# prestodb/presto

Measured on AMD Instinct MI355X. Metric: tpch_lineitem_rows_per_sec, higher is better.
Workload: dtype f64; 1 GPU; TPC-H SF100 Q1 & Q3 on 1xMI355X - one step = one Q1 pass + one Q3 pass, columns resident in HBM; query=q1+q3, rows_per_gpu=1200075804, mode=f64

## Files before the change

### include/presto_gpu.h

```cpp
#ifndef PRESTO_GPU_H
#define PRESTO_GPU_H
#include <stdint.h>

#ifdef __cplusplus
extern "C" {
#endif

#define PG_ABI_VERSION 1

typedef int32_t pg_status;
#define PG_OK 0
#define PG_ERR (-1)
const char* pg_last_error(void);

pg_status pg_device_count(int32_t* out);
pg_status pg_device_sync(void);
pg_status pg_device_malloc(int64_t bytes, void** out);
pg_status pg_device_free(void* p);
pg_status pg_memcpy_h2d(void* dst, const void* src, int64_t bytes);
pg_status pg_memcpy_d2h(void* dst, const void* src, int64_t bytes);
pg_status pg_memcpy_d2d(void* dst, const void* src, int64_t bytes);
double pg_last_hot_kernel_ms(void);
double pg_hot_max_ms(void);
void pg_hot_reset(void);
int64_t pg_q1_fast_launches(void);
int64_t pg_build_staged_launches(void);

typedef enum {
    PG_T_U8 = 0,
    PG_T_I32 = 1,
    PG_T_I64 = 2,
    PG_T_F64 = 3,
    PG_T_I128 = 5,
    PG_T_VARBIN = 4,
} pg_type;

typedef struct {
    int32_t tag;
    int32_t on_device;
    void* data;
    const uint8_t* null_mask;
    const int32_t* offsets;
    const int32_t* dict_ids;
    int32_t dict_n;
} pg_col;

typedef struct {
    int64_t n_rows;
    int32_t n_cols;
    pg_col cols[32];
} pg_page;


typedef enum { PG_CMP_LT = 0, PG_CMP_LE, PG_CMP_GT, PG_CMP_GE, PG_CMP_EQ,
               PG_CMP_NE,
               PG_CMP_CONTAINS, PG_CMP_PREFIX,
               PG_CMP_CONTAINS2, PG_CMP_NOT_CONTAINS2,
               PG_CMP_IS_NULL, PG_CMP_IS_NOT_NULL } pg_cmp;

// ... 230 lines not shown
```

### presto_amd/csrc/kernels.hip

```cpp
#include <hip/hip_runtime.h>
#include <stdio.h>
#include <stdlib.h>
#include <string.h>
#include <map>
#include <vector>
#include <algorithm>
#include <type_traits>
#include <stdexcept>
#include <string>

#include "../../include/presto_gpu.h"
#include "fixed128.h"
#include "sortkey.h"

static __thread char g_err[512];
extern "C" const char* pg_last_error(void) { return g_err; }
static pg_status seterr(const char* msg)
{
    snprintf(g_err, sizeof(g_err), "%s", msg);
    return PG_ERR;
}
#define CHK(x)                                                          \
    do {                                                                \
        hipError_t e_ = (x);                                            \
// ... 87 lines not shown
static hipEvent_t g_ev0, g_ev1;
static bool g_ev_init = false;
static void hot_begin()
{
    hipError_t e;
    if (!g_ev_init) {
        e = hipEventCreate(&g_ev0);
        e = hipEventCreate(&g_ev1);
        g_ev_init = true;
    }
    e = hipEventRecord(g_ev0, g_stream);
    (void)e;
}
static void hot_end()
{
    hipError_t e;
    e = hipEventRecord(g_ev1, g_stream);
    e = hipEventSynchronize(g_ev1);
    float ms = 0;
    e = hipEventElapsedTime(&ms, g_ev0, g_ev1);
    (void)e;
    g_last_hot_ms = ms;
    if (ms > g_hot_max_ms) g_hot_max_ms = ms;
}
extern "C" double pg_last_hot_kernel_ms(void) { return g_last_hot_ms; }
extern "C" double pg_hot_max_ms(void) { return g_hot_max_ms; }
extern "C" void pg_hot_reset(void) { g_hot_max_ms = 0.0; }
static int64_t g_q1_fast_launches = 0;
extern "C" int64_t pg_q1_fast_launches(void) { return g_q1_fast_launches; }
static int64_t g_build_staged_launches = 0;
extern "C" int64_t pg_build_staged_launches(void)
{
    return g_build_staged_launches;
}

#define WAVE 64
#define FT_NBLOCKS 4096
#define FT_NTHREADS 256
#define FT_VL ((int64_t)FT_NBLOCKS * FT_NTHREADS)
static const int64_t TBL_EMPTY = INT64_MIN;

__device__ __host__ inline uint8_t d_tbl_tag(uint64_t h)
{
    return (uint8_t)((h >> 56) | 1);
}

__device__ inline double d_load_f64(const pg_col& c, int64_t i)
{
    switch (c.tag) {
        case PG_T_F64: return ((const double*)c.data)[i];
        case PG_T_I64: return (double)((const int64_t*)c.data)[i];
        case PG_T_I32: return (double)((const int32_t*)c.data)[i];
        default: return (double)((const uint8_t*)c.data)[i];
    }
}
__device__ inline int64_t d_load_i64(const pg_col& c, int64_t i)
{
    switch (c.tag) {
        case PG_T_I64: return ((const int64_t*)c.data)[i];
        case PG_T_I32: return (int64_t)((const int32_t*)c.data)[i];
        case PG_T_U8: return (int64_t)((const uint8_t*)c.data)[i];
        default: return (int64_t)((const double*)c.data)[i];
    }
}

__device__ inline int32_t d_find(const uint8_t* d, int32_t n,
// ... 1592 lines not shown
__device__ inline int64_t d_tbl_find_tagged(const int64_t* keys,
                                            const uint8_t* tags,
                                            int64_t mask, int64_t lmask,
                                            int32_t pbits, int64_t key)
{
    if (!tags) return d_tbl_find(keys, mask, lmask, pbits, key);
    uint64_t h = pg_murmur3_finalize(pg_bigint_hash(key));
    int64_t s = (int64_t)(h & (uint64_t)mask);
    uint8_t tag = d_tbl_tag(h);
    for (;;) {
        uint8_t t = tags[s];
        if (t == 0) return -1;
        if (t == tag && (keys[s] >> pbits) == key) return s;
        s = d_probe_next(s, lmask);
    }
}

struct slot_acc {
    unsigned long long dec;
    unsigned long long flo;
    unsigned long long fhi;
    unsigned long long cnt;
};

__device__ inline void d_atomic_add_dec_ck(unsigned long long* slot,
                                           int64_t ticks,
                                           unsigned long long* ovf)
{
    long long old = (long long)atomicAdd(slot, (unsigned long long)ticks);
    long long nv = old + ticks;
    if (((old ^ nv) & (ticks ^ nv)) < 0 && ovf) atomicAdd(ovf, 1ull);
}

__global__ __launch_bounds__(256) void k_probe_agg(
    pg_page pg, pg_plan_lookup_join plan, const int64_t* keys,
    const uint8_t* tags, int64_t mask, int64_t lmask, int32_t pbits,
    const unsigned long long* kbits, int64_t bmax,
    unsigned long long* acc, int32_t aw,
    unsigned long long* ovf )
{
    const int C = 4;
    int64_t base =
        ((int64_t)blockIdx.x * blockDim.x + threadIdx.x) * C;
    const int64_t stride = (int64_t)gridDim.x * blockDim.x * C;
    for (; base < pg.n_rows; base += stride) {
        const int64_t lim = base + C < pg.n_rows ? base + C : pg.n_rows;
        int64_t cur_key = 0, cur_slot = -2;
        int64_t run_dec = 0;
        long long run_min = INT64_MAX;
        uint64_t run_flo = 0, run_fhi = 0;
        int run_cnt = 0;
        auto flush = [&]() {
            if (cur_slot < 0 || run_cnt == 0) return;
            unsigned long long* s = acc + (size_t)cur_slot * aw;
            if (plan.dec_min) {
                atomicMin((long long*)&s[0], run_min);
            } else if (run_dec) {
                d_atomic_add_dec_ck(&s[0], run_dec, ovf);
            }
            if (!plan.dec_only && !plan.dec_min && (run_flo | run_fhi)) {
                unsigned long long old = atomicAdd(&s[1], run_flo);
                atomicAdd(&s[2],
                          run_fhi + (old > ~run_flo ? 1ull : 0ull));
            }
            atomicAdd(&s[aw - 1], (unsigned long long)run_cnt);
        };
        for (int64_t i = base; i < lim; i++) {
            if (!d_eval_preds(pg, plan.preds, plan.n_preds, i)) continue;
            int64_t key = d_load_i64(pg.cols[plan.key_col], i);
            if (cur_slot == -2 || key != cur_key) {
                flush();
                cur_key = key;
                if (!keys)
                    cur_slot = (uint64_t)(key - 1) <= (uint64_t)mask
                                   ? key - 1
                                   : -1;
                else
                    cur_slot = kbits && !d_kbit_test(kbits, bmax, key)
                                   ? -1
                                   : d_tbl_find_tagged(keys, tags, mask,
                                                       lmask, pbits, key);
                run_dec = 0;
                run_flo = run_fhi = 0;
                run_cnt = 0;
                run_min = INT64_MAX;
            }
            if (cur_slot < 0) continue;
            pg_agg ag;
            ag.proj = plan.proj;
            ag.dec_scale = plan.dec_scale;
            int64_t ticks = d_eval_proj_dec(pg, ag, i);
            if (plan.dec_min) {
                run_min = ticks < run_min ? ticks : run_min;
            } else if (__builtin_add_overflow(run_dec, ticks, &run_dec)) {
                if (ovf) atomicAdd(ovf, 1ull);
            }
            if (!plan.dec_only && !plan.dec_min) {
                double p = d_eval_proj_f64(pg, plan.proj, i);
                uint64_t phi, plo;
                d_fx128_from_f64_ck(p, &phi, &plo, ovf + 1);
                uint64_t nlo = run_flo + plo;
                run_fhi += phi + (nlo < plo ? 1u : 0u);
                run_flo = nlo;
            }
            run_cnt++;
        }
        flush();
    }
}

__global__ __launch_bounds__(256) void k_probe_agg_q3(
    const int32_t* sd , int32_t pred_op,
    int32_t pred_val, const int64_t* okey, const double* ep,
    const double* dc, int64_t n, const int64_t* keys, const uint8_t* tags,
    int64_t mask, int64_t lmask, int32_t pbits,
    const unsigned long long* kbits, int64_t bmax, int32_t dec_only,
    unsigned long long* acc, int32_t aw, unsigned long long* ovf)
{
    typedef int vi2 __attribute__((ext_vector_type(2)));
    typedef long vl2 __attribute__((ext_vector_type(2)));
    const int Q = 2;
    int64_t base0 = Q * ((int64_t)blockIdx.x * blockDim.x + threadIdx.x);
    int64_t stride = Q * (int64_t)gridDim.x * blockDim.x;
    for (int64_t base = base0; base < n; base += stride) {
        int64_t k[Q];
        int32_t s[Q];
        bool sel[Q];
        if (base + Q <= n) {
            vl2 ka = __builtin_nontemporal_load((const vl2*)(okey + base));
            k[0] = ka[0]; k[1] = ka[1];
            if (sd) {
                vi2 ss = __builtin_nontemporal_load((const vi2*)(sd + base));
                s[0] = ss[0]; s[1] = ss[1];
            }
#pragma unroll
            for (int j = 0; j < Q; j++) sel[j] = true;
        } else {
#pragma unroll
            for (int j = 0; j < Q; j++) {
                sel[j] = base + j < n;
                k[j] = sel[j] ? okey[base + j] : 0;
                s[j] = sel[j] && sd ? sd[base + j] : 0;
            }
        }
        if (sd) {
#pragma unroll
            for (int j = 0; j < Q; j++)
                sel[j] = sel[j] && (pred_op == PG_CMP_GT ? s[j] > pred_val
                                                         : s[j] < pred_val);
        }
        int64_t slot[Q];
#pragma unroll
        for (int j = 0; j < Q; j++) {
            slot[j] = -1;
            if (!sel[j]) continue;
            if (kbits && !d_kbit_test(kbits, bmax, k[j])) continue;
            uint64_t h = pg_murmur3_finalize(pg_bigint_hash(k[j]));
            int64_t p = (int64_t)(h & (uint64_t)mask);
            uint8_t tg = tags ? d_tbl_tag(h) : 0;
            for (;;) {
                if (tags) {
                    uint8_t t = tags[p];
                    if (t == 0) break;
                    if (t == tg && (keys[p] >> pbits) == k[j]) {
                        slot[j] = p;
                        break;
                    }
                } else {
                    int64_t kw = keys[p];
                    if (kw == TBL_EMPTY) break;
                    if ((kw >> pbits) == k[j]) { slot[j] = p; break; }
                }
                p = d_probe_next(p, lmask);
            }
        }
#pragma unroll
        for (int j = 0; j < Q; j++) {
            int64_t sl = slot[j];
            if (sl < 0) continue;
            double e = ep[base + j], d = dc[base + j];
            int64_t cents = d_round_ticks(e * 100.0);
            int64_t di = d_round_ticks(d * 100.0);
            int64_t ticks = cents * (100 - di);
            unsigned long long* s = acc + (size_t)sl * aw;
            atomicAdd(&s[0], (unsigned long long)ticks);
            if (!dec_only) {
                double pr = e * (1.0 - d);
                uint64_t phi, plo;
                d_fx128_from_f64_ck(pr, &phi, &plo, ovf + 1);
                unsigned long long old = atomicAdd(&s[1], plo);
                atomicAdd(&s[2], phi + (old > ~plo ? 1ull : 0ull));
            }
            atomicAdd(&s[aw - 1], 1ull);
        }
    }
}

__global__ __launch_bounds__(256) void k_probe_agg_pay(
    pg_page pg, pg_plan_lookup_join plan, const int64_t* keys1,
    const uint8_t* tags1, const int32_t* head1, int64_t mask1,
    int64_t lmask1, const unsigned long long* kbits1, int64_t bmax1,
    const int64_t* pay1, const int64_t* keys2,
    const uint8_t* tags2, int64_t mask2, int64_t lmask2,
    unsigned long long* acc2, int32_t aw, unsigned long long* ovf)
{
    int64_t i = (int64_t)blockIdx.x * blockDim.x + threadIdx.x;
    int64_t stride = (int64_t)gridDim.x * blockDim.x;
    for (; i < pg.n_rows; i += stride) {
        if (!d_eval_preds(pg, plan.preds, plan.n_preds, i)) continue;
        int64_t key = d_load_i64(pg.cols[plan.key_col], i);
        if (kbits1 && !d_kbit_test(kbits1, bmax1, key)) continue;
        int64_t s1 = d_tbl_find_tagged(keys1, tags1, mask1, lmask1, 0,
                                       key);
        if (s1 < 0) continue;
        int64_t r = head1 ? (int64_t)head1[s1] : s1;
        if (r < 0) continue;
        int64_t g = pay1[r];
        int64_t s2 =
            keys2 ? d_tbl_find_tagged(keys2, tags2, mask2, lmask2, 0, g)
                  : ((uint64_t)(g - 1) <= (uint64_t)mask2 ? g - 1 : -1);
        if (s2 < 0) continue;
        pg_agg ag;
        ag.proj = plan.proj;
        ag.dec_scale = plan.dec_scale;
        int64_t ticks = d_eval_proj_dec(pg, ag, i);
        unsigned long long* s = acc2 + (size_t)s2 * aw;
        d_atomic_add_dec_ck(&s[0], ticks, ovf);
        if (!plan.dec_only) {
// ... 823 lines not shown
                (int64_t)s[acc_words - 1];
        }
        __syncthreads();
        if (threadIdx.x == 0)
            running += wcnt[0] + wcnt[1] + wcnt[2] + wcnt[3];
        __syncthreads();
    }
}

__global__ __launch_bounds__(256) void k_groups_count(
    const unsigned long long* acc, int64_t stride_w, int64_t cnt_off,
    int32_t cnt_shift, unsigned long long cnt_mask,
    int64_t cap, int64_t chunk, int64_t* block_counts)
{
    const int64_t lo = (int64_t)blockIdx.x * chunk;
    const int64_t hi = min(lo + chunk, cap);
    const int lane = threadIdx.x & 63, wid = threadIdx.x >> 6;
    int64_t cnt = 0;
    for (int64_t base = lo + 64 * wid; base < hi; base += 256) {
        int64_t i = base + lane;
        bool sel = i < hi &&
                   ((acc[i * stride_w + cnt_off] >> cnt_shift) &
                    cnt_mask) > 0;
        uint64_t m = d_ballot(sel);
        if (lane == 0) cnt += __popcll(m);
    }
    __shared__ int64_t lds[4];
    if (lane == 0) lds[wid] = cnt;
    __syncthreads();
    if (threadIdx.x == 0)
        block_counts[blockIdx.x] = lds[0] + lds[1] + lds[2] + lds[3];
}

__global__ __launch_bounds__(256) void k_groups_emit(
    const int64_t* keys, const int32_t* head,
    const unsigned long long* acc, int32_t aw, build_payloads bp,
    int64_t cap, int64_t chunk, unsigned long long* cursor,
    int64_t* out_key, emit_outs payload_outs, int64_t* out_dec,
    double* out_f64, int64_t* out_cnt)
{
    const int64_t lo = (int64_t)blockIdx.x * chunk;
    const int64_t hi = min(lo + chunk, cap);
    const int lane = threadIdx.x & 63, wid = threadIdx.x >> 6;
    __shared__ int64_t wcnt[4];
    __shared__ int64_t running;
    {
        int64_t mycnt = 0;
        for (int64_t i = lo + threadIdx.x; i < hi; i += 256)
            mycnt += acc[i * aw + aw - 1] > 0;
        mycnt = d_bfly_i64(mycnt);
        if (lane == 0) wcnt[wid] = mycnt;
        __syncthreads();
        if (threadIdx.x == 0)
            running = wcnt[0] + wcnt[1] + wcnt[2] + wcnt[3]
                          ? (int64_t)atomicAdd(
                                cursor, (unsigned long long)(wcnt[0] +
                                                             wcnt[1] +
                                                             wcnt[2] +
                                                             wcnt[3]))
                          : 0;
    }
    __syncthreads();
    for (int64_t base = lo; base < hi; base += 256) {
        int64_t i = base + 64 * wid + lane;
        bool sel = i < hi && acc[i * aw + aw - 1] > 0;
        uint64_t m = d_ballot(sel);
        int wsum = __popcll(m);
        if (lane == 0) wcnt[wid] = wsum;
        __syncthreads();
        int64_t woff = running;
        for (int w = 0; w < wid; w++) woff += wcnt[w];
        if (sel) {
            int64_t pos = woff + __popcll(m & ((1ull << lane) - 1));
            int64_t kw = keys ? keys[i] : i + 1;
            out_key[pos] = bp.pack_bits ? (kw >> bp.pack_bits) : kw;
            int64_t r = bp.by_slot ? i : (int64_t)head[i];
            for (int o = 0; o < bp.n; o++) {
                int64_t pv = bp.pack_bits && o == 0
                                 ? (kw & ((1ll << bp.pack_bits) - 1))
                                 : 0;
                switch (bp.tag[o]) {
                    case PG_T_U8:
                        ((uint8_t*)payload_outs.ptr[o])[pos] =
                            bp.pack_bits && o == 0
                                ? (uint8_t)pv
                                : ((const uint8_t*)bp.ptr[o])[r];
                        break;
                    case PG_T_I32:
                        ((int32_t*)payload_outs.ptr[o])[pos] =
                            bp.pack_bits && o == 0
                                ? (int32_t)pv
                                : ((const int32_t*)bp.ptr[o])[r];
                        break;
                    case PG_T_I64:
                        ((int64_t*)payload_outs.ptr[o])[pos] =
                            bp.pack_bits && o == 0
                                ? pv
                                : ((const int64_t*)bp.ptr[o])[r];
                        break;
                    default:
                        ((double*)payload_outs.ptr[o])[pos] =
                            ((const double*)bp.ptr[o])[r];
                }
            }
            const unsigned long long* s = acc + (size_t)i * aw;
            out_dec[pos] = (int64_t)s[0];
            out_f64[pos] = aw == 4 ? fx128_to_f64(s[2], s[1]) : 0.0;
            out_cnt[pos] = (int64_t)s[aw - 1];
        }
        __syncthreads();
        if (threadIdx.x == 0)
            running += wcnt[0] + wcnt[1] + wcnt[2] + wcnt[3];
        __syncthreads();
    }
}

#define TOPN_NB 256
#define TOPN_MAXL 16

struct topn_cand {
    int64_t val_bits;
    int64_t key;
    int32_t date;
    int32_t valid;
};

__device__ inline bool d_topn_less(bool is_f64, int64_t av, int32_t ad,
                                   int64_t ak, int64_t bv, int32_t bd,
                                   int64_t bk)
{
    if (av != bv) {
        if (is_f64) {
            double x = __longlong_as_double(av), y = __longlong_as_double(bv);
            return x < y;
        }
        return av < bv;
    }
    if (ad != bd) return ad > bd;
    return ak > bk;
}

__global__ __launch_bounds__(256) void k_topn(const void* vals, int is_f64,
                                              const int32_t* dates,
                                              const int64_t* keys, int64_t n,
                                              int32_t L, topn_cand* block_out)
{
    int64_t lv[TOPN_MAXL];
// ... 984 lines not shown
                bufs.emplace_back();
                bufs.back().alloc(n);
                CHKV(hipMemcpyAsync(bufs.back().p, in->cols[c].data, n,
                                    hipMemcpyHostToDevice, g_stream));
                pg.cols[c].data = bufs.back().p;
                pg.cols[c].on_device = 1;
                if (in->cols[c].null_mask) {
                    bufs.emplace_back();
                    bufs.back().alloc(in->n_rows);
                    CHKV(hipMemcpyAsync(bufs.back().p, in->cols[c].null_mask,
                                        in->n_rows, hipMemcpyHostToDevice,
                                        g_stream));
                    pg.cols[c].null_mask = (const uint8_t*)bufs.back().p;
                }
            }
        }
    }
};

struct OutPage {
    pg_page pg{};
    std::vector<DevBuf> dev;
    std::vector<std::vector<uint8_t>> host;
};

struct Table {
    int64_t cap = 0, mask = 0, n_rows = 0;
    int64_t local_mask = 0;
    int32_t pack_bits = 0;
    bool key_set_only = false;
    DevBuf keys, head, next, tags;
    DevBuf acc;
    int32_t acc_words = 0;
    DevBuf acc_multi;
    int32_t n_acc = 0;
    int32_t acc_stride = 0;
    DevBuf kbits;
    int64_t bmax = 0;
    bool range_group = false;
    bool dense_alloc_pending = false;
    bool slot_payloads = false;
    bool dense = false;
    DevBuf key_rows;
    std::vector<DevBuf> payload;
    std::vector<int32_t> ptag;
};

static std::mutex g_mu;
static std::map<int64_t, std::unique_ptr<Table>> g_tables;
static int64_t g_next_table = 1;

struct Op {
    int32_t kind;
    bool finished = false;
    std::deque<OutPage> outq;
    OutPage current;
    virtual void add_input(const pg_page* p) = 0;
    virtual void finish() = 0;
    virtual ~Op() = default;
    virtual int64_t table_handle() { return -1; }
    virtual void partition_counts(int64_t*, int32_t)
    {
        throw std::runtime_error("not a partition op");
    }
    const pg_page* pop_output()
    {
        if (outq.empty()) return nullptr;
        current = std::move(outq.front());
        outq.pop_front();
        return &current.pg;
    }
};

static int64_t next_pow2(int64_t x)
{
    int64_t c = 2;
    while (c < x) c <<= 1;
    return c;
}
// ... 539 lines not shown
        if (semi) {
            const pg_col& sc = pg.cols[plan.semijoin_col];
            if (!semi->dense || semi->ptag.empty() ||
                semi->ptag[0] != PG_T_U8 || !vec_i64(sc))
                return false;
            a.sk = (const int64_t*)sc.data;
            a.flags = (const uint8_t*)semi->payload[0].p;
            a.nflags = semi->cap;
        }
        a.pay_pred = -1;
        if (lu) {
            const pg_col& lc = pg.cols[plan.payload_lookup_key_col];
            if (!lu->dense || !vec_i64(lc)) return false;
            a.lk = (const int64_t*)lc.data;
            a.lu = (const uint8_t*)lu->payload[0].p;
            a.lucap = lu->cap;
        } else {
            const pg_col& pc = pg.cols[plan.payload_col[0]];
            if (pc.tag != PG_T_I32 && pc.tag != PG_T_U8 &&
                pc.tag != PG_T_I64)
                return false;
            a.pay = pc.data;
            a.pay_tag = pc.tag;
            for (int p = 0; p < plan.n_preds; p++)
                if (plan.preds[p].col == plan.payload_col[0]) a.pay_pred = p;
        }
        *sa = a;
        return true;
    }
    void init()
    {
        t.reset(new Table());
        t->key_set_only = plan.key_set_only != 0;
        if (plan.dense_array || plan.agg_table)
            for (int p = 0; p < plan.n_preds && p < PG_MAX_PRED; p++)
                if (plan.preds[p].op >= PG_CMP_IS_NULL)
                    throw std::runtime_error(
                        "IS NULL / IS NOT NULL predicates are not "
                        "supported on dense_array and agg_table builds "
                        "(filter ahead of the build, or use a chained "
                        "build)");
        if (plan.range_group) {
            if (plan.capacity_hint <= 0)
                throw std::runtime_error(
                    "range_group needs capacity_hint = max key");
            t->range_group = true;
            t->slot_payloads = true;
            t->cap = plan.capacity_hint;
            t->mask = t->cap - 1;
            t->local_mask = t->mask;
            return;
        }
        if (plan.dense_array) {
            if (plan.n_payload != 1 && !plan.key_set_only)
                throw std::runtime_error(
                    "dense_array needs one u8 payload (or key_set_only)");
            t->dense = true;
            t->cap = plan.capacity_hint;
            t->payload.emplace_back();
            t->ptag.push_back(PG_T_U8);
            t->dense_alloc_pending = true;
            if (plan.key_set_only) {
                t->payload.back().alloc((size_t)t->cap);
                t->payload.back().zero();
                t->dense_alloc_pending = false;
            }
// ... 535 lines not shown
                    plan.acc_pack_cnt_shift +
                        plan.acc_pack_cnt_width > 64)
                    throw std::runtime_error("acc_pack: bad cnt field");
                for (int a = 0; a < plan.n_aggs; a++) {
                    if (plan.acc_pack_shift[a] < 0) {
                        want_stride++;
                        continue;
                    }
                    if (plan.acc_pack_width[a] < 1 ||
                        plan.acc_pack_shift[a] +
                            plan.acc_pack_width[a] > 64)
                        throw std::runtime_error(
                            "acc_pack: bad field bounds");
                    unsigned long long fm =
                        ((1ull << plan.acc_pack_width[a]) - 1)
                        << plan.acc_pack_shift[a];
                    if (used & fm)
                        throw std::runtime_error(
                            "acc_pack: overlapping fields");
                    used |= fm;
                }
            }
            if (t->acc_multi.p && (t->n_acc != plan.n_aggs ||
                                   t->acc_stride != want_stride))
                throw std::runtime_error(
                    "table already carries a different multi-agg layout");
            if (!t->acc_multi.p) {
                t->n_acc = plan.n_aggs;
                t->acc_stride = want_stride;
                t->acc_multi.alloc((size_t)t->cap * want_stride * 8);
                t->acc_multi.zero();
                CHKV(hipStreamSynchronize(g_stream));
            }
        } else if (plan.mode == 1) {
            int32_t want_aw = (plan.dec_only || plan.dec_min) ? 2 : 4;
            if (!t->acc.p) {
                t->acc_words = want_aw;
                t->acc.alloc((size_t)t->cap * t->acc_words * 8);
                t->acc.zero();
                CHKV(hipStreamSynchronize(g_stream));
            } else if (want_aw == 4 && t->acc_words == 2) {
                throw std::runtime_error(
                    "table accumulators were allocated dec-only; fx128 "
                    "probes need a fresh table");
            }
        }
        if (plan.mode == 1 && plan.dec_min) {
            hipLaunchKernelGGL(k_acc_min_init, dim3(2048), dim3(256), 0,
                               g_stream, (unsigned long long*)t->acc.p,
                               t->acc_words, t->cap);
            CHKV(hipStreamSynchronize(g_stream));
        }
        if (plan.mode == 2) {
            if (!t->slot_payloads || t->ptag.size() != 1 ||
                t->ptag[0] != PG_T_U8)
                throw std::runtime_error(
                    "mode 2 probes an agg_table with one u8 payload");
            auto it2 = g_tables.find(plan.table2);
            if (it2 == g_tables.end() || !it2->second->dense)
                throw std::runtime_error("mode 2 needs a dense_array "
                                         "table2");
            t2 = it2->second.get();
            if (plan.n_group_vals < 1 || plan.n_group_vals > 8)
                throw std::runtime_error("n_group_vals must be 1..8");
            m2_acc.alloc(4 * 8 * 8 + 8);
            m2_acc.zero();
        }
        if (plan.mode == 3) {
            if (t->slot_payloads || t->ptag.empty() ||
                t->ptag[0] != PG_T_I64)
                throw std::runtime_error(
                    "mode 3 needs a chained build whose first payload "
                    "is the i64 grouping key");
            auto it2 = g_tables.find(plan.table2);
            if (it2 == g_tables.end() || it2->second->dense ||
                it2->second->key_set_only)
                throw std::runtime_error(
                    "mode 3 needs an agg/keyed table2 for the groups");
            t2 = it2->second.get();
            if (t2->pack_bits)
                throw std::runtime_error(
                    "mode 3 groups table cannot be packed");
            if (!t2->acc.p) {
                t2->acc_words = 4;
                t2->acc.alloc((size_t)t2->cap * 4 * 8);
                t2->acc.zero();
                CHKV(hipStreamSynchronize(g_stream));
            }
        }
    }
    void add_input(const pg_page* in) override
    {
        StagedPage sp;
        sp.stage(in);
        if (plan.mode == 2) {
            unsigned long long* a = (unsigned long long*)m2_acc.p;
            bool spec = plan.n_preds == 0 && t->pack_bits > 0 &&
                        plan.proj.kind == PG_PROJ_DISC_PRICE &&
                        sp.pg.cols[plan.key_col].tag == PG_T_I64 &&
                        sp.pg.cols[plan.table2_key_col].tag == PG_T_I64 &&
                        sp.pg.cols[plan.proj.a].tag == PG_T_F64 &&
                        sp.pg.cols[plan.proj.b].tag == PG_T_F64 &&
                        plan.dec_scale == 4 &&
                        !((uintptr_t)sp.pg.cols[plan.key_col].data & 15) &&
                        !((uintptr_t)sp.pg.cols[plan.table2_key_col].data &
                          15) &&
                        !sp.pg.cols[plan.key_col].null_mask &&
                        !sp.pg.cols[plan.table2_key_col].null_mask &&
                        !sp.pg.cols[plan.proj.a].null_mask &&
                        !sp.pg.cols[plan.proj.b].null_mask;
            hot_begin();
            if (spec) {
                hipLaunchKernelGGL(
                    k_probe_agg_q5<8>, dim3(4096), dim3(256), 0, g_stream,
                    plan, (const int64_t*)sp.pg.cols[plan.key_col].data,
                    (const int64_t*)sp.pg.cols[plan.table2_key_col].data,
                    (const double*)sp.pg.cols[plan.proj.a].data,
                    (const double*)sp.pg.cols[plan.proj.b].data,
                    sp.pg.n_rows, (const int64_t*)t->keys.p,
                    (const uint8_t*)t->tags.p, t->mask, t->local_mask,
                    t->pack_bits, (const unsigned long long*)t->kbits.p, t->bmax,
                    (const uint8_t*)t2->payload[0].p,
                    t2->cap, a, a + 8, a + 16, a + 24);
            } else {
                hipLaunchKernelGGL(k_probe_agg_fused2<8>, dim3(4096),
                                   dim3(256), 0, g_stream, sp.pg, plan,
                                   (const int64_t*)t->keys.p,
                                   t->local_mask, t->pack_bits,
                                   (const uint8_t*)t->tags.p, t->mask,
                                   (const uint8_t*)t->payload[0].p,
                                   (const uint8_t*)t2->payload[0].p,
                                   t2->cap, a, a + 8, a + 16, a + 24);
            }
            hot_end();
            CHKV(hipStreamSynchronize(g_stream));
            return;
        }
        if (plan.mode == 3) {
            hot_begin();
            hipLaunchKernelGGL(k_probe_agg_pay, dim3(4096), dim3(256), 0,
                               g_stream, sp.pg, plan,
                               (const int64_t*)t->keys.p,
                               (const uint8_t*)t->tags.p,
                               (const int32_t*)t->head.p, t->mask,
                               t->local_mask,
                               (const unsigned long long*)t->kbits.p, t->bmax,
                               (const int64_t*)t->payload[0].p,
                               (const int64_t*)t2->keys.p,
                               (const uint8_t*)t2->tags.p, t2->mask,
                               t2->local_mask,
                               (unsigned long long*)t2->acc.p,
                               t2->acc_words,
                               (unsigned long long*)ovf.p);
            hot_end();
            CHKV(hipStreamSynchronize(g_stream));
            return;
        }
        if (plan.mode == 1 && plan.n_aggs > 0) {
            hot_begin();
            hipLaunchKernelGGL(k_probe_agg_multi, dim3(4096), dim3(256), 0,
                               g_stream, sp.pg, plan,
                               (const int64_t*)t->keys.p,
                               (const uint8_t*)t->tags.p, t->mask,
                               t->local_mask, t->pack_bits,
                               (const unsigned long long*)t->kbits.p, t->bmax,
                               (unsigned long long*)t->acc_multi.p,
                               (unsigned long long*)ovf.p);
            hot_end();
            CHKV(hipStreamSynchronize(g_stream));
            return;
        }
// ... 5 lines not shown
                        sp.pg.cols[plan.proj.b].tag == PG_T_F64 &&
                        plan.dec_scale == 4 && plan.n_preds <= 1 &&
                        !((uintptr_t)sp.pg.cols[plan.key_col].data & 15) &&
                        !((uintptr_t)sp.pg.cols[plan.proj.a].data & 15) &&
                        !((uintptr_t)sp.pg.cols[plan.proj.b].data & 15);
            if (plan.n_preds == 1) {
                const pg_pred& pr = plan.preds[0];
                spec = spec && pr.rhs_col == 0 &&
                       sp.pg.cols[pr.col].tag == PG_T_I32 &&
                       (pr.op == PG_CMP_GT || pr.op == PG_CMP_LT) &&
                       !((uintptr_t)sp.pg.cols[pr.col].data & 7) &&
                       !sp.pg.cols[pr.col].null_mask;
            }
            spec = spec && !sp.pg.cols[plan.key_col].null_mask &&
                   !sp.pg.cols[plan.proj.a].null_mask &&
                   !sp.pg.cols[plan.proj.b].null_mask;
            hot_begin();
            if (spec) {
                const pg_pred& pr = plan.preds[0];
                hipLaunchKernelGGL(
                    k_probe_agg_q3, dim3(4096), dim3(256), 0, g_stream,
                    plan.n_preds
                        ? (const int32_t*)sp.pg.cols[pr.col].data
                        : nullptr,
                    plan.n_preds ? pr.op : 0,
                    plan.n_preds ? (int32_t)pr.ival : 0,
                    (const int64_t*)sp.pg.cols[plan.key_col].data,
                    (const double*)sp.pg.cols[plan.proj.a].data,
                    (const double*)sp.pg.cols[plan.proj.b].data,
                    sp.pg.n_rows, (const int64_t*)t->keys.p,
                    (const uint8_t*)t->tags.p, t->mask, t->local_mask,
                    t->pack_bits, (const unsigned long long*)t->kbits.p, t->bmax, plan.dec_only,
                    (unsigned long long*)t->acc.p, t->acc_words,
                    (unsigned long long*)ovf.p);
            } else {
                hipLaunchKernelGGL(k_probe_agg, dim3(4096), dim3(256), 0,
                                   g_stream, sp.pg, plan,
                                   (const int64_t*)t->keys.p,
                                   (const uint8_t*)t->tags.p, t->mask,
                                   t->local_mask, t->pack_bits,
                                   (const unsigned long long*)t->kbits.p, t->bmax,
                                   (unsigned long long*)t->acc.p,
                                   t->acc_words,
                                   (unsigned long long*)ovf.p);
            }
            hot_end();
            CHKV(hipStreamSynchronize(g_stream));
            return;
        }
        int64_t n = sp.pg.n_rows;
        if (outer()) {
            for (int o = 0; o < plan.n_emit; o++)
                if (sp.pg.cols[plan.emit_probe_cols[o]].tag == PG_T_VARBIN)
                    throw std::runtime_error(
                        "outer LOOKUP_JOIN emits fixed-width probe "
                        "columns only");
            if (probe_tags.empty())
                for (int o = 0; o < plan.n_emit; o++)
                    probe_tags.push_back(
                        sp.pg.cols[plan.emit_probe_cols[o]].tag);
        }
        if (n == 0) {
            OutPage op;
            op.pg.n_rows = 0;
            op.pg.n_cols = plan.n_emit + (int32_t)t->payload.size();
            for (int c = 0; c < op.pg.n_cols; c++) {
                op.pg.cols[c].tag = PG_T_I64;
                if (outer())
                    op.pg.cols[c].tag =
                        c < plan.n_emit ? probe_tags[c]
                                        : payload_tag(t, c - plan.n_emit);
                op.pg.cols[c].on_device = 1;
                op.pg.cols[c].data = nullptr;
            }
            outq.push_back(std::move(op));
            return;
        }
        const uint8_t* dv8 = (const uint8_t*)(
            t->dense && t->ptag[0] == PG_T_U8 ? t->payload[0].p : nullptr);
// ... 136 lines not shown
        OutPage op;
        op.pg.n_rows = r.n;
        op.pg.n_cols = plan.n_emit + np;
        op.dev.emplace_back();
        op.dev.back().alloc((size_t)r.n);
        uint8_t* ones = (uint8_t*)op.dev.back().p;
        CHKV(hipMemsetAsync(ones, 1, op.dev.back().sz, g_stream));
        for (int o = 0; o < plan.n_emit; o++) {
            int tag = probe_tags.empty() ? PG_T_I64 : probe_tags[o];
            op.dev.emplace_back();
            op.dev.back().alloc((size_t)r.n * type_size(tag));
            op.dev.back().zero();
            op.pg.cols[o].tag = tag;
            op.pg.cols[o].on_device = 1;
            op.pg.cols[o].data = op.dev.back().p;
            op.pg.cols[o].null_mask = ones;
        }
        emit_outs outs{};
        outs.n = np;
        for (int o = 0; o < np; o++) {
            int tag = payload_tag(t, o);
            op.dev.emplace_back();
            op.dev.back().alloc((size_t)r.n * type_size(tag));
            pg_col& c = op.pg.cols[plan.n_emit + o];
            c.tag = tag;
            c.on_device = 1;
            c.data = op.dev.back().p;
            outs.ptr[o] = c.data;
            outs.tag[o] = tag;
        }
        sel_emit(bpg, fp, nullptr, 0, chunk, r, outs);
        outq.push_back(std::move(op));
    }
    void finish() override
    {
        if (marking()) {
            drain();
            return;
        }
        if (plan.mode == 2) {
            unsigned long long h[33];
            CHKV(hipMemcpy(h, m2_acc.p, sizeof(h), hipMemcpyDeviceToHost));
            if (h[32])
                throw std::runtime_error(
                    "decimal SUM overflow in fused probe "
                    "(Math.addExact semantics)");
            int n_out = 0;
            for (int g = 0; g < plan.n_group_vals; g++)
                if (h[24 + g]) n_out++;
            OutPage op;
            op.pg.n_rows = n_out;
            op.pg.n_cols = 4;
            op.host.emplace_back(n_out ? n_out : 1);
            op.host.emplace_back((size_t)(n_out ? n_out : 1) * 8);
            op.host.emplace_back((size_t)(n_out ? n_out : 1) * 8);
            op.host.emplace_back((size_t)(n_out ? n_out : 1) * 8);
            op.pg.cols[0].tag = PG_T_U8;
            op.pg.cols[1].tag = PG_T_I64;
            op.pg.cols[2].tag = PG_T_F64;
            op.pg.cols[3].tag = PG_T_I64;
            for (int c = 0; c < 4; c++) {
                op.pg.cols[c].on_device = 0;
                op.pg.cols[c].data = op.host[c].data();
            }
            int row = 0;
            for (int g = 0; g < plan.n_group_vals; g++) {
                if (!h[24 + g]) continue;
                ((uint8_t*)op.pg.cols[0].data)[row] = plan.group_vals[g];
                ((int64_t*)op.pg.cols[1].data)[row] = (int64_t)h[g];
                ((double*)op.pg.cols[2].data)[row] =
                    fx128_to_f64(h[16 + g], h[8 + g]);
                ((int64_t*)op.pg.cols[3].data)[row] = (int64_t)h[24 + g];
                row++;
            }
            outq.push_back(std::move(op));
            return;
        }
        if (plan.mode != 1 && plan.mode != 3) return;
        {
            unsigned long long h_ovf[2] = {0, 0};
            CHKV(hipMemcpy(h_ovf, ovf.p, 16, hipMemcpyDeviceToHost));
            if (h_ovf[0])
                throw std::runtime_error(
                    "bigint/decimal SUM overflow in grouped probe "
                    "(Math.addExact semantics, "
                    "LongSumAggregation.java:33-37)");
            if (h_ovf[1])
                throw std::runtime_error(
                    "SUM_F64 addend outside the exact fixed-point domain "
                    "in grouped probe (needs 0 <= x < 2^53 with no "
                    "fraction bits below 2^-64)");
        }
        Table* gt = plan.mode == 3 ? t2 : t;
        const bool multi = plan.mode == 1 && plan.n_aggs > 0;
        int64_t cap = gt->cap;
        int64_t chunk = (cap + FLT_NB - 1) / FLT_NB;
        chunk = (chunk + 255) / 256 * 256;
        if (chunk < 256) chunk = 256;
        int64_t total = gt->n_rows;
        if (gt->range_group) {
            DevBuf d_counts;
            d_counts.alloc(FLT_NB * 8);
            const unsigned long long* cacc =
                multi ? (const unsigned long long*)gt->acc_multi.p
                      : (const unsigned long long*)gt->acc.p;
            int64_t stride_w =
                multi ? gt->acc_stride : gt->acc_words;
            int64_t cnt_off = stride_w - 1;
            int32_t cnt_shift = 0;
            unsigned long long cnt_mask = ~0ull;
            if (multi && plan.acc_pack) {
                cnt_off = 0;
                cnt_shift = plan.acc_pack_cnt_shift;
                cnt_mask = (1ull << plan.acc_pack_cnt_width) - 1;
            }
            hipLaunchKernelGGL(k_groups_count, dim3(FLT_NB), dim3(256),
                               0, g_stream, cacc, stride_w, cnt_off,
                               cnt_shift, cnt_mask,
                               cap, chunk, (int64_t*)d_counts.p);
            std::vector<int64_t> hc(FLT_NB);
            CHKV(hipMemcpyAsync(hc.data(), d_counts.p, FLT_NB * 8,
                                hipMemcpyDeviceToHost, g_stream));
            CHKV(hipStreamSynchronize(g_stream));
            total = 0;
// ... 1140 lines not shown
    *out = t;
    return PG_OK;
}
extern "C" pg_status pg_op_partition_counts(pg_op h, int64_t* counts,
                                            int32_t n)
{
    auto op = find_op(h);
    if (!op) return seterr("bad op handle");
    try {
        op->partition_counts(counts, n);
        return PG_OK;
    } catch (std::exception& e) {
        return seterr(e.what());
    }
}
extern "C" pg_status pg_table_destroy(int64_t t)
{
    std::lock_guard<std::mutex> lk(g_mu);
    g_tables.erase(t);
    return PG_OK;
}

extern "C" pg_status pg_table_reset_acc(int64_t t)
{
    try {
        Table* tbl;
        {
            std::lock_guard<std::mutex> lk(g_mu);
            auto it = g_tables.find(t);
            if (it == g_tables.end())
                return seterr("pg_table_reset_acc: table not found");
            tbl = it->second.get();
        }
        if (tbl->acc.p)
            CHK(hipMemsetAsync(tbl->acc.p, 0, tbl->acc.sz, g_stream));
        if (tbl->acc_multi.p)
            CHK(hipMemsetAsync(tbl->acc_multi.p, 0, tbl->acc_multi.sz,
                               g_stream));
        CHK(hipStreamSynchronize(g_stream));
        return PG_OK;
    } catch (const std::exception& e) {
        return seterr(e.what());
    }
}

namespace {

static uint32_t crc32_tab_[256];
static bool crc32_init_ = false;
static uint32_t pg_crc32(uint32_t crc, const uint8_t* p, size_t n)
{
    if (!crc32_init_) {
        for (uint32_t i = 0; i < 256; i++) {
            uint32_t c = i;
            for (int k = 0; k < 8; k++)
                c = (c & 1) ? 0xEDB88320u ^ (c >> 1) : c >> 1;
            crc32_tab_[i] = c;
        }
        crc32_init_ = true;
    }
    crc = ~crc;
    for (size_t i = 0; i < n; i++)
        crc = crc32_tab_[(crc ^ p[i]) & 0xff] ^ (crc >> 8);
    return ~crc;
}

struct ByteWriter {
    uint8_t* p;
// ... 583 lines not shown
```

Before: 123.0 billion rows/s.

## Record first-touched group slots during probe to extract groups by list

The grouped probe kernels (including the Q3 path) now append each accumulator slot to a device-side hit list the first time its count goes from zero, staging entries per wave in LDS and flushing with one atomic per wave. At finish, when the list is small relative to the accumulator table, a list-driven emit kernel writes only the touched groups instead of scanning and compacting the whole table. This removes the full-table scan in Q3 group extraction. In exchange it adds ballot and LDS work plus extra atomics to the hot probe loop, and sets occupancy hints on the probe kernels.

New measurement: 136.7 billion rows/s (median of 6 runs). 11.2% higher.

```diff
diff --git a/include/presto_gpu.h b/include/presto_gpu.h
--- a/include/presto_gpu.h
+++ b/include/presto_gpu.h
@@ -25,6 +25,7 @@
 void pg_hot_reset(void);
 int64_t pg_q1_fast_launches(void);
 int64_t pg_build_staged_launches(void);
+int64_t pg_groups_list_extractions(void);
 
 typedef enum {
     PG_T_U8 = 0,
diff --git a/presto_amd/csrc/kernels.hip b/presto_amd/csrc/kernels.hip
--- a/presto_amd/csrc/kernels.hip
+++ b/presto_amd/csrc/kernels.hip
@@ -143,6 +143,11 @@
 extern "C" int64_t pg_build_staged_launches(void)
 {
     return g_build_staged_launches;
+}
+static int64_t g_groups_list_extractions = 0;
+extern "C" int64_t pg_groups_list_extractions(void)
+{
+    return g_groups_list_extractions;
 }
 
 #define WAVE 64
@@ -1801,20 +1806,74 @@
     if (((old ^ nv) & (ticks ^ nv)) < 0 && ovf) atomicAdd(ovf, 1ull);
 }
 
-__global__ __launch_bounds__(256) void k_probe_agg(
+struct hit_list {
+    void* ents;
+    unsigned long long* cursor;
+    int64_t cap;
+    int32_t wide;
+};
+
+__device__ inline void d_hits_flush(const hit_list& hl,
+                                    volatile int64_t* wbuf, int cnt)
+{
+    const int lane = threadIdx.x & 63;
+    int64_t g = 0;
+    __builtin_amdgcn_fence(__ATOMIC_RELEASE, "wavefront");
+    __builtin_amdgcn_wave_barrier();
+    if (lane == 0)
+        g = (int64_t)atomicAdd(hl.cursor, (unsigned long long)cnt);
+    g = __shfl(g, 0, WAVE);
+    if (lane < cnt && g + lane < hl.cap) {
+        int64_t s = wbuf[lane];
+        if (hl.wide)
+            ((int64_t*)hl.ents)[g + lane] = s;
+        else
+            ((uint32_t*)hl.ents)[g + lane] = (uint32_t)s;
+    }
+    __builtin_amdgcn_fence(__ATOMIC_ACQUIRE, "wavefront");
+    __builtin_amdgcn_wave_barrier();
+}
+
+__device__ inline void d_hits_stage(const hit_list& hl,
+                                    volatile int64_t* wbuf, int* cnt,
+                                    bool ft, int64_t slot)
+{
+    uint64_t m = d_ballot(ft);
+    if (!m) return;
+    const int lane = threadIdx.x & 63;
+    int pos = *cnt + __popcll(m & ((1ull << lane) - 1));
+    int total = *cnt + __popcll(m);
+    if (ft && pos < WAVE) wbuf[pos] = slot;
+    if (total >= WAVE) {
+        d_hits_flush(hl, wbuf, WAVE);
+        if (ft && pos >= WAVE) wbuf[pos - WAVE] = slot;
+        total -= WAVE;
+    }
+    *cnt = total;
+}
+
+__global__ __launch_bounds__(256)
+__attribute__((amdgpu_waves_per_eu(7))) void k_probe_agg(
     pg_page pg, pg_plan_lookup_join plan, const int64_t* keys,
     const uint8_t* tags, int64_t mask, int64_t lmask, int32_t pbits,
     const unsigned long long* kbits, int64_t bmax,
     unsigned long long* acc, int32_t aw,
-    unsigned long long* ovf )
+    unsigned long long* ovf ,
+    hit_list hl)
 {
     const int C = 4;
     int64_t base =
         ((int64_t)blockIdx.x * blockDim.x + threadIdx.x) * C;
     const int64_t stride = (int64_t)gridDim.x * blockDim.x * C;
-    for (; base < pg.n_rows; base += stride) {
+    const int lane = threadIdx.x & 63;
+    __shared__ int64_t hbuf[4][WAVE];
+    volatile int64_t* wbuf = hbuf[threadIdx.x >> 6];
+    int hcnt = 0;
+    for (; base - C * lane < pg.n_rows; base += stride) {
         const int64_t lim = base + C < pg.n_rows ? base + C : pg.n_rows;
         int64_t cur_key = 0, cur_slot = -2;
+        int64_t fts[C] = {0, 0, 0, 0};
+        int nft = 0;
         int64_t run_dec = 0;
         long long run_min = INT64_MAX;
         uint64_t run_flo = 0, run_fhi = 0;
@@ -1832,7 +1891,14 @@
                 atomicAdd(&s[2],
                           run_fhi + (old > ~run_flo ? 1ull : 0ull));
             }
-            atomicAdd(&s[aw - 1], (unsigned long long)run_cnt);
+            unsigned long long old =
+                atomicAdd(&s[aw - 1], (unsigned long long)run_cnt);
+            if (old == 0 && hl.ents) {
+#pragma unroll
+                for (int k = C - 1; k > 0; k--) fts[k] = fts[k - 1];
+                fts[0] = cur_slot;
+                nft++;
+            }
         };
         for (int64_t i = base; i < lim; i++) {
             if (!d_eval_preds(pg, plan.preds, plan.n_preds, i)) continue;
@@ -1875,23 +1941,43 @@
             run_cnt++;
         }
         flush();
-    }
-}
-
-__global__ __launch_bounds__(256) void k_probe_agg_q3(
+        if (hl.ents) {
+#pragma unroll
+            for (int k = 0; k < C; k++)
+                d_hits_stage(hl, wbuf, &hcnt, k < nft, fts[k]);
+        }
+    }
+    if (hl.ents && hcnt) d_hits_flush(hl, wbuf, hcnt);
+}
+
+__global__ __launch_bounds__(256)
+__attribute__((amdgpu_waves_per_eu(8))) void k_probe_agg_q3(
     const int32_t* sd , int32_t pred_op,
     int32_t pred_val, const int64_t* okey, const double* ep,
     const double* dc, int64_t n, const int64_t* keys, const uint8_t* tags,
     int64_t mask, int64_t lmask, int32_t pbits,
     const unsigned long long* kbits, int64_t bmax, int32_t dec_only,
-    unsigned long long* acc, int32_t aw, unsigned long long* ovf)
+    unsigned long long* acc, int32_t aw, unsigned long long* ovf,
+    hit_list hl)
 {
     typedef int vi2 __attribute__((ext_vector_type(2)));
     typedef long vl2 __attribute__((ext_vector_type(2)));
     const int Q = 2;
     int64_t base0 = Q * ((int64_t)blockIdx.x * blockDim.x + threadIdx.x);
     int64_t stride = Q * (int64_t)gridDim.x * blockDim.x;
-    for (int64_t base = base0; base < n; base += stride) {
+    const int lane = threadIdx.x & 63;
+    __shared__ int64_t hbuf[4][WAVE];
+    volatile int64_t* wbuf = hbuf[threadIdx.x >> 6];
+    int hcnt = 0;
+    int64_t pslot[Q];
+    unsigned long long pold[Q];
+#pragma unroll
+    for (int j = 0; j < Q; j++) {
+        pslot[j] = -1;
+        pold[j] = 1;
+    }
+    for (int64_t base = base0; base - Q * lane < n + stride;
+         base += stride) {
         int64_t k[Q];
         int32_t s[Q];
         bool sel[Q];
@@ -1943,9 +2029,16 @@
                 p = d_probe_next(p, lmask);
             }
         }
+        if (hl.ents) {
+#pragma unroll
+            for (int j = 0; j < Q; j++)
+                d_hits_stage(hl, wbuf, &hcnt,
+                             pslot[j] >= 0 && pold[j] == 0, pslot[j]);
+        }
 #pragma unroll
         for (int j = 0; j < Q; j++) {
             int64_t sl = slot[j];
+            pslot[j] = sl;
             if (sl < 0) continue;
             double e = ep[base + j], d = dc[base + j];
             int64_t cents = d_round_ticks(e * 100.0);
@@ -1960,9 +2053,10 @@
                 unsigned long long old = atomicAdd(&s[1], plo);
                 atomicAdd(&s[2], phi + (old > ~plo ? 1ull : 0ull));
             }
-            atomicAdd(&s[aw - 1], 1ull);
-        }
-    }
+            pold[j] = atomicAdd(&s[aw - 1], 1ull);
+        }
+    }
+    if (hl.ents && hcnt) d_hits_flush(hl, wbuf, hcnt);
 }
 
 __global__ __launch_bounds__(256) void k_probe_agg_pay(
@@ -2852,6 +2946,49 @@
         block_counts[blockIdx.x] = lds[0] + lds[1] + lds[2] + lds[3];
 }
 
+__device__ inline void d_group_row(
+    const int64_t* keys, const int32_t* head,
+    const unsigned long long* acc, int32_t aw, const build_payloads& bp,
+    int64_t i, int64_t pos, int64_t* out_key, const emit_outs& payload_outs,
+    int64_t* out_dec, double* out_f64, int64_t* out_cnt)
+{
+    int64_t kw = keys ? keys[i] : i + 1;
+    out_key[pos] = bp.pack_bits ? (kw >> bp.pack_bits) : kw;
+    int64_t r = bp.by_slot ? i : (int64_t)head[i];
+    for (int o = 0; o < bp.n; o++) {
+        int64_t pv = bp.pack_bits && o == 0
+                         ? (kw & ((1ll << bp.pack_bits) - 1))
+                         : 0;
+        switch (bp.tag[o]) {
+            case PG_T_U8:
+                ((uint8_t*)payload_outs.ptr[o])[pos] =
+                    bp.pack_bits && o == 0
+                        ? (uint8_t)pv
+                        : ((const uint8_t*)bp.ptr[o])[r];
+                break;
+            case PG_T_I32:
+                ((int32_t*)payload_outs.ptr[o])[pos] =
+                    bp.pack_bits && o == 0
+                        ? (int32_t)pv
+                        : ((const int32_t*)bp.ptr[o])[r];
+                break;
+            case PG_T_I64:
+                ((int64_t*)payload_outs.ptr[o])[pos] =
+                    bp.pack_bits && o == 0
+                        ? pv
+                        : ((const int64_t*)bp.ptr[o])[r];
+                break;
+            default:
+                ((double*)payload_outs.ptr[o])[pos] =
+                    ((const double*)bp.ptr[o])[r];
+        }
+    }
+    const unsigned long long* s = acc + (size_t)i * aw;
+    out_dec[pos] = (int64_t)s[0];
+    out_f64[pos] = aw == 4 ? fx128_to_f64(s[2], s[1]) : 0.0;
+    out_cnt[pos] = (int64_t)s[aw - 1];
+}
+
 __global__ __launch_bounds__(256) void k_groups_emit(
     const int64_t* keys, const int32_t* head,
     const unsigned long long* acc, int32_t aw, build_payloads bp,
@@ -2892,47 +3029,28 @@
         for (int w = 0; w < wid; w++) woff += wcnt[w];
         if (sel) {
             int64_t pos = woff + __popcll(m & ((1ull << lane) - 1));
-            int64_t kw = keys ? keys[i] : i + 1;
-            out_key[pos] = bp.pack_bits ? (kw >> bp.pack_bits) : kw;
-            int64_t r = bp.by_slot ? i : (int64_t)head[i];
-            for (int o = 0; o < bp.n; o++) {
-                int64_t pv = bp.pack_bits && o == 0
-                                 ? (kw & ((1ll << bp.pack_bits) - 1))
-                                 : 0;
-                switch (bp.tag[o]) {
-                    case PG_T_U8:
-                        ((uint8_t*)payload_outs.ptr[o])[pos] =
-                            bp.pack_bits && o == 0
-                                ? (uint8_t)pv
-                                : ((const uint8_t*)bp.ptr[o])[r];
-                        break;
-                    case PG_T_I32:
-                        ((int32_t*)payload_outs.ptr[o])[pos] =
-                            bp.pack_bits && o == 0
-                                ? (int32_t)pv
-                                : ((const int32_t*)bp.ptr[o])[r];
-                        break;
-                    case PG_T_I64:
-                        ((int64_t*)payload_outs.ptr[o])[pos] =
-                            bp.pack_bits && o == 0
-                                ? pv
-                                : ((const int64_t*)bp.ptr[o])[r];
-                        break;
-                    default:
-                        ((double*)payload_outs.ptr[o])[pos] =
-                            ((const double*)bp.ptr[o])[r];
-                }
-            }
-            const unsigned long long* s = acc + (size_t)i * aw;
-            out_dec[pos] = (int64_t)s[0];
-            out_f64[pos] = aw == 4 ? fx128_to_f64(s[2], s[1]) : 0.0;
-            out_cnt[pos] = (int64_t)s[aw - 1];
+            d_group_row(keys, head, acc, aw, bp, i, pos, out_key,
+                        payload_outs, out_dec, out_f64, out_cnt);
         }
         __syncthreads();
         if (threadIdx.x == 0)
             running += wcnt[0] + wcnt[1] + wcnt[2] + wcnt[3];
         __syncthreads();
     }
+}
+
+__global__ __launch_bounds__(256) void k_groups_emit_list(
+    const void* hits, int32_t wide, int64_t n_hits, const int64_t* keys,
+    const int32_t* head, const unsigned long long* acc, int32_t aw,
+    build_payloads bp, int64_t* out_key, emit_outs payload_outs,
+    int64_t* out_dec, double* out_f64, int64_t* out_cnt)
+{
+    int64_t pos = (int64_t)blockIdx.x * blockDim.x + threadIdx.x;
+    if (pos >= n_hits) return;
+    int64_t i = wide ? ((const int64_t*)hits)[pos]
+                     : (int64_t)((const uint32_t*)hits)[pos];
+    d_group_row(keys, head, acc, aw, bp, i, pos, out_key, payload_outs,
+                out_dec, out_f64, out_cnt);
 }
 
 #define TOPN_NB 256
@@ -3983,6 +4101,11 @@
     DevBuf keys, head, next, tags;
     DevBuf acc;
     int32_t acc_words = 0;
+    DevBuf hits, hits_n;
+    int64_t hits_cap = 0;
+    unsigned long long hits_n_host = 0;
+    bool use_hits = true;
+    bool list_ok = false;
     DevBuf acc_multi;
     int32_t n_acc = 0;
     int32_t acc_stride = 0;
@@ -3996,6 +4119,26 @@
     std::vector<DevBuf> payload;
     std::vector<int32_t> ptag;
 };
+
+static void hits_restart(Table* t)
+{
+    if (!t->hits.p) return;
+    CHKV(hipMemsetAsync(t->hits_n.p, 0, 8, g_stream));
+    t->hits_n_host = 0;
+    t->list_ok = true;
+}
+
+static hit_list hits_arg(const Table* t)
+{
+    hit_list hl{};
+    if (t->list_ok) {
+        hl.ents = t->hits.p;
+        hl.cursor = (unsigned long long*)t->hits_n.p;
+        hl.cap = t->hits_cap;
+        hl.wide = t->cap > (1ll << 32);
+    }
+    return hl;
+}
 
 static std::mutex g_mu;
 static std::map<int64_t, std::unique_ptr<Table>> g_tables;
@@ -4601,6 +4744,8 @@
     {
         t.reset(new Table());
         t->key_set_only = plan.key_set_only != 0;
+        if (const char* eg = getenv("PG_GROUPS_LIST"))
+            t->use_hits = atoi(eg) != 0;
         if (plan.dense_array || plan.agg_table)
             for (int p = 0; p < plan.n_preds && p < PG_MAX_PRED; p++)
                 if (plan.preds[p].op >= PG_CMP_IS_NULL)
@@ -5202,12 +5347,22 @@
                 t->acc_multi.zero();
                 CHKV(hipStreamSynchronize(g_stream));
             }
+            t->list_ok = false;
         } else if (plan.mode == 1) {
             int32_t want_aw = (plan.dec_only || plan.dec_min) ? 2 : 4;
             if (!t->acc.p) {
                 t->acc_words = want_aw;
                 t->acc.alloc((size_t)t->cap * t->acc_words * 8);
                 t->acc.zero();
+                if (t->use_hits && !t->range_group) {
+                    t->hits_cap = t->n_rows;
+                    t->hits.alloc((size_t)t->hits_cap *
+                                  (t->cap > (1ll << 32) ? 8 : 4));
+                    t->hits_n.alloc(8);
+                    t->hits_n.zero();
+                    t->hits_n_host = 0;
+                    t->list_ok = true;
+                }
                 CHKV(hipStreamSynchronize(g_stream));
             } else if (want_aw == 4 && t->acc_words == 2) {
                 throw std::runtime_error(
@@ -5219,6 +5374,7 @@
             hipLaunchKernelGGL(k_acc_min_init, dim3(2048), dim3(256), 0,
                                g_stream, (unsigned long long*)t->acc.p,
                                t->acc_words, t->cap);
+            hits_restart(t);
             CHKV(hipStreamSynchronize(g_stream));
         }
         if (plan.mode == 2) {
@@ -5257,6 +5413,7 @@
                 t2->acc.zero();
                 CHKV(hipStreamSynchronize(g_stream));
             }
+            t2->list_ok = false;
         }
     }
     void add_input(const pg_page* in) override
@@ -5307,6 +5464,7 @@
             return;
         }
         if (plan.mode == 3) {
+            t2->list_ok = false;
             hot_begin();
             hipLaunchKernelGGL(k_probe_agg_pay, dim3(4096), dim3(256), 0,
                                g_stream, sp.pg, plan,
@@ -5378,7 +5536,7 @@
                     (const uint8_t*)t->tags.p, t->mask, t->local_mask,
                     t->pack_bits, (const unsigned long long*)t->kbits.p, t->bmax, plan.dec_only,
                     (unsigned long long*)t->acc.p, t->acc_words,
-                    (unsigned long long*)ovf.p);
+                    (unsigned long long*)ovf.p, hits_arg(t));
             } else {
                 hipLaunchKernelGGL(k_probe_agg, dim3(4096), dim3(256), 0,
                                    g_stream, sp.pg, plan,
@@ -5388,9 +5546,12 @@
                                    (const unsigned long long*)t->kbits.p, t->bmax,
                                    (unsigned long long*)t->acc.p,
                                    t->acc_words,
-                                   (unsigned long long*)ovf.p);
+                                   (unsigned long long*)ovf.p, hits_arg(t));
             }
             hot_end();
+            if (t->list_ok)
+                CHKV(hipMemcpyAsync(&t->hits_n_host, t->hits_n.p, 8,
+                                    hipMemcpyDeviceToHost, g_stream));
             CHKV(hipStreamSynchronize(g_stream));
             return;
         }
@@ -5593,6 +5754,51 @@
         sel_emit(bpg, fp, nullptr, 0, chunk, r, outs);
         outq.push_back(std::move(op));
     }
+    void extract_by_list(OutPage& op)
+    {
+        const int64_t total = (int64_t)t->hits_n_host;
+        op.pg.n_rows = total;
+        int nc = 0;
+        auto add_dev_col = [&](int tag) {
+            op.dev.emplace_back();
+            op.dev.back().alloc((size_t)total * type_size(tag));
+            op.pg.cols[nc].tag = tag;
+            op.pg.cols[nc].on_device = 1;
+            op.pg.cols[nc].data = op.dev.back().p;
+            return nc++;
+        };
+        int c_key = add_dev_col(PG_T_I64);
+        build_payloads bp{};
+        bp.n = (int32_t)t->payload.size();
+        bp.by_slot = t->slot_payloads ? 1 : 0;
+        bp.pack_bits = t->pack_bits;
+        emit_outs pl_outs{};
+        pl_outs.n = bp.n;
+        for (int o = 0; o < bp.n; o++) {
+            bp.ptr[o] = t->payload[o].p;
+            bp.tag[o] = t->ptag[o];
+            int c = add_dev_col(t->ptag[o]);
+            pl_outs.ptr[o] = op.pg.cols[c].data;
+            pl_outs.tag[o] = t->ptag[o];
+        }
+        int c_dec = add_dev_col(PG_T_I64);
+        int c_f64 = add_dev_col(PG_T_F64);
+        int c_cnt = add_dev_col(PG_T_I64);
+        op.pg.n_cols = nc;
+        if (total == 0) return;
+        hipLaunchKernelGGL(k_groups_emit_list,
+                           dim3((unsigned)((total + 255) / 256)), dim3(256),
+                           0, g_stream, (const void*)t->hits.p,
+                           (int32_t)(t->cap > (1ll << 32)), total,
+                           (const int64_t*)t->keys.p,
+                           (const int32_t*)t->head.p,
+                           (const unsigned long long*)t->acc.p,
+                           t->acc_words, bp,
+                           (int64_t*)op.pg.cols[c_key].data, pl_outs,
+                           (int64_t*)op.pg.cols[c_dec].data,
+                           (double*)op.pg.cols[c_f64].data,
+                           (int64_t*)op.pg.cols[c_cnt].data);
+    }
     void finish() override
     {
         if (marking()) {
@@ -5638,9 +5844,18 @@
             return;
         }
         if (plan.mode != 1 && plan.mode != 3) return;
+        OutPage lop;
+        const bool by_list =
+            plan.mode == 1 && plan.n_aggs == 0 && t->list_ok &&
+            !t->range_group && t->hits_n_host <= (uint64_t)t->hits_cap &&
+            (double)t->hits_n_host * 128.0 <
+                (double)t->cap * t->acc_words * 8.0;
+        if (by_list) extract_by_list(lop);
         {
             unsigned long long h_ovf[2] = {0, 0};
-            CHKV(hipMemcpy(h_ovf, ovf.p, 16, hipMemcpyDeviceToHost));
+            CHKV(hipMemcpyAsync(h_ovf, ovf.p, 16, hipMemcpyDeviceToHost,
+                                g_stream));
+            CHKV(hipStreamSynchronize(g_stream));
             if (h_ovf[0])
                 throw std::runtime_error(
                     "bigint/decimal SUM overflow in grouped probe "
@@ -5651,6 +5866,11 @@
                     "SUM_F64 addend outside the exact fixed-point domain "
                     "in grouped probe (needs 0 <= x < 2^53 with no "
                     "fraction bits below 2^-64)");
+        }
+        if (by_list) {
+            g_groups_list_extractions++;
+            outq.push_back(std::move(lop));
+            return;
         }
         Table* gt = plan.mode == 3 ? t2 : t;
         const bool multi = plan.mode == 1 && plan.n_aggs > 0;
@@ -6857,8 +7077,10 @@
                 return seterr("pg_table_reset_acc: table not found");
             tbl = it->second.get();
         }
-        if (tbl->acc.p)
+        if (tbl->acc.p) {
             CHK(hipMemsetAsync(tbl->acc.p, 0, tbl->acc.sz, g_stream));
+            hits_restart(tbl);
+        }
         if (tbl->acc_multi.p)
             CHK(hipMemsetAsync(tbl->acc_multi.p, 0, tbl->acc_multi.sz,
                                g_stream));
```
